# JuanDuGit/DH3D

Hardware: AMD Instinct MI355X
Metric: point-clouds/sec (higher is better)
Workload: dtype f32; 1 GPU; local-descriptor forward (basic_config), N=8192 K=8, batch=8; clouds_per_gpu=8, clouds_total=8, points=8192, knn=8, parallelism=clouds sharded over 1 GPU(s), no data-path collective, weights=random-init (no checkpoint blobs exist upstream), steps_in_flight=4

## Files before the change

### dh3d_amd/csrc/spatial.hip

```cpp
#include <math.h>

#include "cell_grid.h"
#include "common.h"
#include "wave_ops.h"

namespace {

constexpr int kThreads = 1024;
constexpr int kWaves = 16;

__device__ __forceinline__ unsigned spread6(unsigned v) {
  v &= 63u;
  v = (v | (v << 8)) & 0x300Fu;
  v = (v | (v << 4)) & 0x30C3u;
  v = (v | (v << 2)) & 0x9249u;
  return v;
}
constexpr unsigned kSchedCube = 0x186186u;

__device__ __forceinline__ unsigned deal_grid_bits(const float ext[3], int nb[3]) {
  float c0 = ext[0], c1 = ext[1], c2 = ext[2];
  int n0 = 0, n1 = 0, n2 = 0;
  unsigned sched = 0;
#pragma unroll
  for (int s = 0; s < 12; ++s) {
    int a = -1;
    float best = -1.f;
    if (n2 < 6) { a = 2; best = c2; }
    if (n1 < 6 && (a < 0 || c1 > best * 1.25f)) { best = a < 0 ? c1 : fmaxf(best, c1); a = 1; }
    if (n0 < 6 && (a < 0 || c0 > best * 1.25f)) { best = a < 0 ? c0 : fmaxf(best, c0); a = 0; }
    n0 += (int)(a == 0); n1 += (int)(a == 1); n2 += (int)(a == 2);
    c0 = a == 0 ? c0 * 0.5f : c0; c1 = a == 1 ? c1 * 0.5f : c1; c2 = a == 2 ? c2 * 0.5f : c2;
    sched |= (unsigned)a << (2 * s);
  }
  nb[0] = n0; nb[1] = n1; nb[2] = n2;
  return sched;
}

template <int PPT>
__global__ __launch_bounds__(kThreads) void spatial_sort_kernel(const float *__restrict__ xyz, int N,
                                                               int npad, float4 *__restrict__ sorted,
                                                               float *__restrict__ gbox, int *__restrict__ cells,
                                                               int occ_min) {
  extern __shared__ __attribute__((aligned(16))) unsigned s_raw[];
  unsigned *s_hist = s_raw + 2 * npad;
  float *s_red = reinterpret_cast<float *>(s_hist + kWaves * 64);
  unsigned *s_tab = reinterpret_cast<unsigned *>(s_red + 6 * kWaves);
  const int b = blockIdx.x, tid = threadIdx.x, lane = tid & 63;
  const int wave = __builtin_amdgcn_readfirstlane(tid >> 6);
  const float *pc = xyz + (size_t)b * N * 3;
  const int NG = (N + 63) / 64;

  const int SEG = npad / kWaves;
  float lo[3] = {INFINITY, INFINITY, INFINITY}, hi[3] = {-INFINITY, -INFINITY, -INFINITY};
  float px[PPT], py[PPT], pz[PPT];
#pragma unroll
  for (int j = 0; j < PPT; ++j) {
    const int k = min(wave * SEG + j * 64 + lane, N - 1);
    px[j] = pc[(size_t)k * 3]; py[j] = pc[(size_t)k * 3 + 1]; pz[j] = pc[(size_t)k * 3 + 2];
  }
#pragma unroll
  for (int j = 0; j < PPT; ++j) {
    lo[0] = fminf(lo[0], px[j]); hi[0] = fmaxf(hi[0], px[j]);
    lo[1] = fminf(lo[1], py[j]); hi[1] = fmaxf(hi[1], py[j]);
    lo[2] = fminf(lo[2], pz[j]); hi[2] = fmaxf(hi[2], pz[j]);
  }
#pragma unroll
  for (int a = 0; a < 3; ++a) {
    const float wl = wave_min_f32(lo[a]), wh = wave_max_f32(hi[a]);
    if (lane == 0) { s_red[wave * 6 + a] = wl; s_red[wave * 6 + 3 + a] = wh; }
  }
  __syncthreads();
  float scale[3], ext[3];
#pragma unroll
  for (int a = 0; a < 3; ++a) {
    float l = INFINITY, h = -INFINITY;
    for (int w = 0; w < kWaves; ++w) { l = fminf(l, s_red[w * 6 + a]); h = fmaxf(h, s_red[w * 6 + 3 + a]); }
    lo[a] = l;
    ext[a] = h - l;
  }
  int nb[3];
  const unsigned sched = deal_grid_bits(ext, nb);
#pragma unroll
  for (int a = 0; a < 3; ++a) scale[a] = (float)(4 << nb[a]) / fmaxf(ext[a], 1e-30f);
  if (cells && tid == 0) {
    int *ct = cells + (size_t)b * kCellInts;
    float *hd = reinterpret_cast<float *>(ct) + kCellHead;
    hd[0] = lo[0]; hd[1] = lo[1]; hd[2] = lo[2];
    hd[3] = scale[0]; hd[4] = scale[1]; hd[5] = scale[2];
    ct[kCellSched] = (int)sched;
  }
  const bool cube = sched == kSchedCube;
  if (!cube) {
    if (tid < 768) {
      const int a = tid >> 8;
      s_tab[tid] = cell_deposit(sched, a, tid & 255, 18, nb[a] + 2, 17);
    }
    __syncthreads();
  }
  constexpr bool RELOAD = PPT >= 16;
  unsigned key[PPT];
  const int q0 = (4 << nb[0]) - 1, q1 = (4 << nb[1]) - 1, q2 = (4 << nb[2]) - 1;
#pragma unroll
  for (int j0 = 0; j0 < PPT; j0 += 4) {
    float rx[4], ry[4], rz[4];
#pragma unroll
    for (int u = 0; u < 4; ++u) {
      if (j0 + u >= PPT) continue;
      if (RELOAD) {
        const int k = min(wave * SEG + (j0 + u) * 64 + lane, N - 1);
        rx[u] = pc[(size_t)k * 3]; ry[u] = pc[(size_t)k * 3 + 1]; rz[u] = pc[(size_t)k * 3 + 2];
      } else {
        rx[u] = px[j0 + u]; ry[u] = py[j0 + u]; rz[u] = pz[j0 + u];
      }
    }
#pragma unroll
    for (int u = 0; u < 4; ++u) {
      if (j0 + u >= PPT) continue;
      const int k = wave * SEG + (j0 + u) * 64 + lane;
      const unsigned cx = (unsigned)min(q0, max(0, (int)((rx[u] - lo[0]) * scale[0])));
      const unsigned cy = (unsigned)min(q1, max(0, (int)((ry[u] - lo[1]) * scale[1])));
      const unsigned cz = (unsigned)min(q2, max(0, (int)((rz[u] - lo[2]) * scale[2])));
      const unsigned cell = cube ? spread6(cx) | (spread6(cy) << 1) | (spread6(cz) << 2)
                                 : s_tab[cx] | s_tab[256 + cy] | s_tab[512 + cz];
      key[j0 + u] = k < N ? (cell << 14) | (unsigned)k : 0xFFFFFFFFu;
    }
    if (RELOAD) __builtin_amdgcn_sched_barrier(0);
  }
  unsigned *src = s_raw, *dst = s_raw + npad;
  const unsigned long long lt_mask = (1ull << lane) - 1ull;
  for (int pass = 0; pass < 3; ++pass) {
    const int shift = 14 + 6 * pass;
    s_hist[tid] = 0u;
    __syncthreads();
    unsigned local[PPT];
    unsigned *whist = s_hist + wave * 64;
#pragma unroll
    for (int j = 0; j < PPT; ++j) {
      const unsigned d = (key[j] >> shift) & 63u;
      unsigned long long same = ~0ull;
#pragma unroll
      for (int i = 0; i < 6; ++i) {
        const bool bit = (d >> i) & 1u;
        const unsigned long long bal = __ballot(bit);
        same &= bit ? bal : ~bal;
      }
      const unsigned before = whist[d];
      const unsigned rank = (unsigned)__popcll(same & lt_mask);
      local[j] = before + rank;
      if (rank == 0) whist[d] = before + (unsigned)__popcll(same);
    }
    __syncthreads();
    {
      const int d = tid >> 4, w = tid & 15;
      const unsigned v = s_hist[w * 64 + d];
      unsigned inc = v;
#pragma unroll
      for (int off = 1; off < 64; off <<= 1) {
        const unsigned up = __shfl_up(inc, off, 64);
        if (lane >= off) inc += up;
      }
      __syncthreads();
      if (lane == 63) s_red[wave] = __uint_as_float(inc);
      __syncthreads();
      unsigned base = 0;
      for (int ww = 0; ww < wave; ++ww) base += __float_as_uint(s_red[ww]);
      s_hist[w * 64 + d] = base + inc - v;
    }
    __syncthreads();
#pragma unroll
    for (int j = 0; j < PPT; ++j) {
      const unsigned d = (key[j] >> shift) & 63u;
      dst[whist[d] + local[j]] = key[j];
    }
    __syncthreads();
#pragma unroll
    for (int j = 0; j < PPT; ++j) key[j] = dst[wave * SEG + j * 64 + lane];
    unsigned *t = src; src = dst; dst = t;
  }
  const unsigned *s_keys = src;
  float gx[PPT], gy[PPT], gz[PPT];
  int gk[PPT];
#pragma unroll
  for (int j = 0; j < PPT; ++j) {
    const int i = min((wave + kWaves * j) * 64 + lane, N - 1);
    gk[j] = (int)(s_keys[i] & 0x3FFFu);
  }
#pragma unroll
  for (int j = 0; j < PPT; ++j) {
    gx[j] = pc[(size_t)gk[j] * 3]; gy[j] = pc[(size_t)gk[j] * 3 + 1]; gz[j] = pc[(size_t)gk[j] * 3 + 2];
  }
#pragma unroll
  for (int j = 0; j < PPT; ++j) {
    const int g = wave + kWaves * j;
    const int i = g * 64 + lane;
    const float x = gx[j], y = gy[j], z = gz[j];
    float lx = INFINITY, ly = INFINITY, lz = INFINITY, hx = -INFINITY, hy = -INFINITY, hz = -INFINITY;
    if (i < N) {
      sorted[(size_t)b * N + i] = make_float4(x, y, z, __int_as_float(gk[j]));
      lx = hx = x; ly = hy = y; lz = hz = z;
    }
    if (g < NG) {
      lx = wave_min_f32(lx); ly = wave_min_f32(ly); lz = wave_min_f32(lz);
      hx = wave_max_f32(hx); hy = wave_max_f32(hy); hz = wave_max_f32(hz);
      if (lane == 0) {
        float *o = gbox + ((size_t)b * NG + g) * 8;
        o[0] = lx; o[1] = ly; o[2] = lz; o[3] = 0.f; o[4] = hx; o[5] = hy; o[6] = hz; o[7] = 0.f;
      }
    }
  }
  if (cells) {
    int *ct = cells + (size_t)b * kCellInts;
#pragma unroll
    for (int j = 0; j < PPT; ++j) {
      const int i = wave * SEG + j * 64 + lane;
      if (i < N) {
        const int cur = (int)(s_keys[i] >> 20), prev = i > 0 ? (int)(s_keys[i - 1] >> 20) : -1;
        for (int c = prev + 1; c <= cur; ++c) ct[c] = i;
        if (i == N - 1)
          for (int c = cur + 1; c <= kGridCells; ++c) ct[c] = N;
      }
    }
    int occupied = 0;
#pragma unroll
    for (int j = 0; j < PPT; ++j) {
      const int i = wave * SEG + j * 64 + lane;
      if (i < N) occupied += (int)(i == 0 || (s_keys[i] >> 20) != (s_keys[i - 1] >> 20));
    }
#pragma unroll
    for (int off = 32; off > 0; off >>= 1) occupied += __shfl_xor(occupied, off, 64);
    __shared__ int s_occupied;
    if (tid == 0) s_occupied = 0;
    __syncthreads();
    if (lane == 0) atomicAdd(&s_occupied, occupied);
    __syncthreads();
    if (tid == 0) ct[kCellFlag] = s_occupied < occ_min ? 1 : 0;
  }
}

template <int PPT>
int sort_launch(const float *xyz, int B, int N, float4 *sorted, float *gbox, int *cells, hipStream_t s) {
  int npad = 2;
  while (npad < N) npad <<= 1;
  if (npad < 64 * kWaves) npad = 64 * kWaves;
  const size_t lds = sizeof(unsigned) * (2 * (size_t)npad + kWaves * 64 + 3 * 256) + sizeof(float) * 6 * kWaves;
  DH3D_ALLOW_BIG_LDS((spatial_sort_kernel<PPT>));
  const int occ_min = (int)(0.6 * kGridCells * (1.0 - exp(-(double)N / kGridCells)));
  hipLaunchKernelGGL((spatial_sort_kernel<PPT>), dim3(B), dim3(kThreads), lds, s, xyz, N, npad, sorted, gbox, cells,
                     occ_min);
  return dh3d_launch_status();
}

}

static int spatial_sort_any(const float *xyz, int B, int N, float *sorted, float *gbox, int *cells, void *stream) {
  DH3D_REQUIRE(xyz && sorted && gbox && B > 0 && N > 0);
  DH3D_SUPPORTED(N <= 16384);
  hipStream_t s = (hipStream_t)stream;
  float4 *so = reinterpret_cast<float4 *>(sorted);
  if (N <= 1024) return sort_launch<1>(xyz, B, N, so, gbox, cells, s);
  if (N <= 2048) return sort_launch<2>(xyz, B, N, so, gbox, cells, s);
  if (N <= 4096) return sort_launch<4>(xyz, B, N, so, gbox, cells, s);
  if (N <= 8192) return sort_launch<8>(xyz, B, N, so, gbox, cells, s);
  return sort_launch<16>(xyz, B, N, so, gbox, cells, s);
}

DH3D_API int dh3d_spatial_sort(const float *xyz, int B, int N, float *sorted, float *gbox, void *stream) {
  return spatial_sort_any(xyz, B, N, sorted, gbox, nullptr, stream);
}

DH3D_API int dh3d_spatial_sort_cells(const float *xyz, int B, int N, float *sorted, float *gbox, int32_t *cells, void *stream) {
  DH3D_REQUIRE(cells);
  return spatial_sort_any(xyz, B, N, sorted, gbox, cells, stream);
}
```

### dh3d_amd/csrc/flex_x6.hip

```cpp
#include <type_traits>

#include "bf16x3.h"

namespace {

typedef float f32x2 __attribute__((ext_vector_type(2)));
typedef float f32x4 __attribute__((ext_vector_type(4)));
constexpr int kTM = 32;
constexpr int kPPR = 32;
constexpr int kProducers = 8 * 64, kThreads = kProducers + 256;

template <int DIN, int DOUT>
struct X6Cfg {
  static constexpr int KD = 4 * DIN;
  static constexpr int LD = KD + 8;
  static constexpr int KB = KD / 16;
  static constexpr int KBH = KB / 2;
  static constexpr int VEC = DIN / 16;
  static constexpr int ROUNDS = kTM / kPPR;
  static constexpr int A_ELEMS = 3 * kTM * LD;
  static constexpr int P_FLOATS = 4 * 8 * 64;
  static constexpr int B3_VEC = 2 * KB * 64;
  static constexpr size_t LDS_BYTES = (size_t)2 * A_ELEMS * 2 + (size_t)2 * P_FLOATS * 4 + (size_t)B3_VEC * 16;
  static_assert(DOUT == 64 && (VEC == 2 || VEC == 4) && KBH % 2 == 0 && LDS_BYTES <= 159 * 1024, "shape");
};

__device__ __forceinline__ void wg_barrier(int = 0) { asm volatile("s_waitcnt lgkmcnt(0)\n\ts_barrier" ::: "memory"); }

template <int K>
__device__ __forceinline__ float row_bcast(float v) {
  return __builtin_bit_cast(float, __builtin_amdgcn_mov_dpp(__builtin_bit_cast(int, v), 0x150 + K, 0xf, 0xf, false));
}

__device__ __forceinline__ float hi16_of(float a) { return __uint_as_float(__float_as_uint(a) & 0xFFFF0000u); }

__device__ __forceinline__ void split3x2(const f32x2 v, unsigned &c1, unsigned &c2, unsigned &c3) {
  const float r0 = v[0] - hi16_of(v[0]), r1 = v[1] - hi16_of(v[1]);
  const float t0 = r0 - hi16_of(r0), t1 = r1 - hi16_of(r1);
  c1 = pack_hi16(v[0], v[1]);
  c2 = pack_hi16(r0, r1);
  c3 = pack_hi16(t0, t1);
}

template <int VEC> struct LaneVec;
template <> struct LaneVec<4> { typedef float4 type; };
template <> struct LaneVec<2> { typedef float2 type; };

template <int DIN, int DOUT, bool RAGGED>
__global__ __launch_bounds__(kThreads) void flex_conv_x6_kernel(
    const float *__restrict__ feat, const float *__restrict__ xyz, const int32_t *__restrict__ nbr,
    const uint4 *__restrict__ wp3, unsigned R, unsigned N, EpilogueArgs ep, float *__restrict__ out, int T) {
  using C = X6Cfg<DIN, DOUT>;
  using FV = typename LaneVec<C::VEC>::type;
  extern __shared__ __attribute__((aligned(16))) unsigned char s_raw[];
  unsigned short *s_A = reinterpret_cast<unsigned short *>(s_raw);
  float *s_P = reinterpret_cast<float *>(s_raw + (size_t)2 * C::A_ELEMS * 2);
  const int tid = threadIdx.x;
  const int wave = __builtin_amdgcn_readfirstlane(tid >> 6);
  const int x = blockIdx.x & 7, slot = blockIdx.x >> 3, S = gridDim.x >> 3;
  const int Tx = (T + 7) >> 3;
  const int tbeg = x * Tx + slot;
  const int tend = (x + 1) * Tx < T ? (x + 1) * Tx : T;
  const int cnt = tbeg < tend ? (tend - tbeg + S - 1) / S : 0;
  if (cnt == 0) return;

  if (wave < kProducers / 64) {
    __builtin_amdgcn_s_setprio(3);
    const int prow = tid >> 4, lj = tid & 15;
    const int c0 = lj * C::VEC;
    const unsigned mrec = (unsigned)(0x100000000ULL / N);
    const int G = cnt * C::ROUNDS;
    int nid[2][8], myid[2][2];
    FV fv[2][8];
    float qd[2][2], pcd[2];
    const int da = (tid >> 2) & 3, di = tid & 3;
    const int dcomp = di > 0 ? di - 1 : 0;

    auto row_of = [&](int g, unsigned &n, bool &ok) {
      const int i = g / C::ROUNDS, r = g % C::ROUNDS;
      n = (unsigned)(tbeg + i * S) * kTM + r * kPPR + prow;
      ok = (int)(g < G) & (int)(n < R);
      n = ok ? n : 0u;
    };
    auto issue_ids = [&](int s, int g) {
      unsigned n; bool ok;
      row_of(g, n, ok);
      const int4 *ip = reinterpret_cast<const int4 *>(nbr + (size_t)n * 8);
      const int4 a = ip[0], b = ip[1];
      nid[s][0] = a.x; nid[s][1] = a.y; nid[s][2] = a.z; nid[s][3] = a.w;
      nid[s][4] = b.x; nid[s][5] = b.y; nid[s][6] = b.z; nid[s][7] = b.w;
      myid[s][0] = nbr[(size_t)n * 8 + da];
      myid[s][1] = nbr[(size_t)n * 8 + 4 + da];
    };
    auto issue_feat = [&](int s, int g) {
      unsigned n; bool ok;
      row_of(g, n, ok);
      unsigned q = __umulhi(n, mrec);
      if (n - q * N >= N) ++q;
      const unsigned cloud0 = q * N;
      pcd[s] = xyz[(size_t)n * 3 + dcomp];
      qd[s][0] = *reinterpret_cast<const float *>(reinterpret_cast<const char *>(xyz) + (size_t)((cloud0 + (unsigned)myid[s][0]) * 12u + (unsigned)dcomp * 4u));
      qd[s][1] = *reinterpret_cast<const float *>(reinterpret_cast<const char *>(xyz) + (size_t)((cloud0 + (unsigned)myid[s][1]) * 12u + (unsigned)dcomp * 4u));
#pragma unroll
      for (int k = 0; k < 8; ++k) {
        const unsigned g2 = cloud0 + (unsigned)nid[s][k];
        fv[s][k] = *reinterpret_cast<const FV *>(reinterpret_cast<const char *>(feat) +
                                                 (size_t)(g2 * (unsigned)(DIN * 4) + (unsigned)(c0 * 4)));
      }
    };
    auto compute = [&](int s, int g) {
      const int i = g / C::ROUNDS, r = g % C::ROUNDS;
      float d0 = qd[s][0] - pcd[s], d1 = qd[s][1] - pcd[s];
      asm volatile("s_nop 1" : "+v"(d0), "+v"(d1));
      f32x2 acc[4][C::VEC / 2];
#define DH3D_X6_FMAC_BCAST(ACC, D, F, L) \
  asm("v_fmac_f32_dpp %0, %1, %2 row_newbcast:" #L " row_mask:0xf bank_mask:0xf" : "+v"(ACC) : "v"(D), "v"(F))
#define DH3D_X6_MUL_BCAST(ACC, D, F, L) \
  asm("v_mul_f32_dpp %0, %1, %2 row_newbcast:" #L " row_mask:0xf bank_mask:0xf" : "=v"(ACC) : "v"(D), "v"(F))
#define DH3D_X6_NEIGHBOUR_(KI, DS, LX, LY, LZ)                                                                   \
  {                                                                                                              \
    const float *fp = reinterpret_cast<const float *>(&fv[s][KI]);                                               \
    _Pragma("unroll") for (int h = 0; h < C::VEC / 2; ++h) {                                                     \
      _Pragma("unroll") for (int e = 0; e < 2; ++e) {                                                            \
        const float f = fp[2 * h + e];                                                                           \
        if ((KI) == 0) {                                                    \
          acc[0][h][e] = f;                                                                                      \
          DH3D_X6_MUL_BCAST(acc[1][h][e], DS, f, LX);                                                            \
          DH3D_X6_MUL_BCAST(acc[2][h][e], DS, f, LY);                                                            \
          DH3D_X6_MUL_BCAST(acc[3][h][e], DS, f, LZ);                                                            \
        } else {                                                                                                 \
          acc[0][h][e] += f;                                                                                     \
          DH3D_X6_FMAC_BCAST(acc[1][h][e], DS, f, LX);                                                           \
          DH3D_X6_FMAC_BCAST(acc[2][h][e], DS, f, LY);                                                           \
          DH3D_X6_FMAC_BCAST(acc[3][h][e], DS, f, LZ);                                                           \
        }                                                                                                        \
      }                                                                                                          \
    }                                                                                                            \
  }
#define DH3D_X6_NEIGHBOUR(KI)                                                                                    \
  if (((KI) & 3) == 0) DH3D_X6_NEIGHBOUR_(KI, ((KI) < 4 ? d0 : d1), 1, 2, 3)                                      \
  else if (((KI) & 3) == 1) DH3D_X6_NEIGHBOUR_(KI, ((KI) < 4 ? d0 : d1), 5, 6, 7)                                 \
  else if (((KI) & 3) == 2) DH3D_X6_NEIGHBOUR_(KI, ((KI) < 4 ? d0 : d1), 9, 10, 11)                               \
  else DH3D_X6_NEIGHBOUR_(KI, ((KI) < 4 ? d0 : d1), 13, 14, 15)
      DH3D_X6_NEIGHBOUR(0) DH3D_X6_NEIGHBOUR(1) DH3D_X6_NEIGHBOUR(2) DH3D_X6_NEIGHBOUR(3)
      DH3D_X6_NEIGHBOUR(4) DH3D_X6_NEIGHBOUR(5) DH3D_X6_NEIGHBOUR(6) DH3D_X6_NEIGHBOUR(7)
#undef DH3D_X6_NEIGHBOUR
#undef DH3D_X6_NEIGHBOUR_
#undef DH3D_X6_FMAC_BCAST
#undef DH3D_X6_MUL_BCAST
      unsigned short *row = s_A + (size_t)(i & 1) * C::A_ELEMS + (size_t)(r * kPPR + prow) * C::LD + c0;
#pragma unroll
      for (int c = 0; c < 4; ++c) {
        unsigned c1[C::VEC / 2], c2[C::VEC / 2], c3[C::VEC / 2];
#pragma unroll
        for (int h = 0; h < C::VEC / 2; ++h) {
          split3x2(acc[c][h], c1[h], c2[h], c3[h]);
        }
        if (C::VEC == 4) {
          *reinterpret_cast<uint2 *>(row + c * DIN) = make_uint2(c1[0], c1[C::VEC / 2 - 1]);
          *reinterpret_cast<uint2 *>(row + c * DIN + kTM * C::LD) = make_uint2(c2[0], c2[C::VEC / 2 - 1]);
          *reinterpret_cast<uint2 *>(row + c * DIN + 2 * kTM * C::LD) = make_uint2(c3[0], c3[C::VEC / 2 - 1]);
        } else {
          *reinterpret_cast<unsigned *>(row + c * DIN) = c1[0];
          *reinterpret_cast<unsigned *>(row + c * DIN + kTM * C::LD) = c2[0];
          *reinterpret_cast<unsigned *>(row + c * DIN + 2 * kTM * C::LD) = c3[0];
        }
      }
    };

    if ((wave >> 2) & 1) {
      issue_ids(0, 0);
      issue_ids(1, 1);
      issue_feat(0, 0);
      issue_ids(0, 2);
      for (int g = 0; g < G; g += 2) {
#pragma unroll
        for (int s = 0; s < 2; ++s) {
          const int gg = g + s;
          issue_feat(s ^ 1, gg + 1);
          issue_ids(s ^ 1, gg + 3);
          compute(s, gg);
          if (gg % C::ROUNDS == C::ROUNDS - 1 && gg < G) wg_barrier(gg / C::ROUNDS);
        }
      }
    } else {
      issue_ids(0, 0);
      issue_ids(1, 1);
      issue_feat(0, 0);
      issue_ids(0, 2);
      issue_feat(1, 1);
      issue_ids(1, 3);
      for (int g = 0; g < G; g += 2) {
#pragma unroll
        for (int s = 0; s < 2; ++s) {
          const int gg = g + s;
          compute(s, gg);
          issue_feat(s, gg + 2);
          issue_ids(s, gg + 4);
          if (gg % C::ROUNDS == C::ROUNDS - 1 && gg < G) wg_barrier(gg / C::ROUNDS);
        }
      }
    }
    wg_barrier(cnt);
  } else {
    const int cw = wave - kProducers / 64, lane = tid & 63;
    const int cb = cw & 1, kh = cw >> 1;
    uint4 breg[C::KBH][2];
    uint4 *const s_b3 = reinterpret_cast<uint4 *>(s_raw + (size_t)2 * C::A_ELEMS * 2 + (size_t)2 * C::P_FLOATS * 4) +
                        (size_t)(cb * C::KB + kh * C::KBH) * 64 + lane;
#pragma unroll
    for (int kb = 0; kb < C::KBH; ++kb) {
#pragma unroll
      for (int p = 0; p < 2; ++p)
        breg[kb][p] = wp3[((size_t)(cb * C::KB + kh * C::KBH + kb) * 3 + p) * 64 + lane];
      s_b3[(size_t)kb * 64] = wp3[((size_t)(cb * C::KB + kh * C::KBH + kb) * 3 + 2) * 64 + lane];
    }
    const int col = cb * 32 + (lane & 31);
    float sc = 1.f, sh = 0.f;
    if (ep.scale) sc = ep.scale[col];
    if (ep.shift) sh = ep.shift[col];
    if (ep.pre_bias) sh = fmaf(ep.pre_bias[col], sc, sh);
    const int lo = ep.act == DH3D_ACT_RELU ? 0 : INT_MIN;
    float4 *const s_P4 = reinterpret_cast<float4 *>(s_P);
    float4 *const p_mine = s_P4 + (size_t)(cw * 2) * 64 + lane;
    const float4 *const p_partner = s_P4 + (size_t)((cw ^ 2) * 2) * 64 + lane;
    const unsigned voff = (unsigned)(((4 * (lane >> 5) + 16 * kh) * DOUT + col) * 4);
    float keep[8];
    const unsigned short *const abase0 = s_A + (size_t)(lane & 31) * C::LD + 8 * (lane >> 5) + kh * C::KBH * 16;

    auto tile = [&](int i, auto prev_tag) {
      constexpr bool PREV = decltype(prev_tag)::value;
      const unsigned short *abase = abase0 + (size_t)(i & 1) * C::A_ELEMS;
      f32x16 acc0, acc1;
#pragma unroll
      for (int r = 0; r < 16; ++r) acc0[r] = acc1[r] = 0.f;
      bf16x8 a[2][3];
      uint4 b3r[2];
      float4 pp[2];
#pragma unroll
      for (int p = 0; p < 3; ++p) a[0][p] = *reinterpret_cast<const bf16x8 *>(abase + p * kTM * C::LD);
      b3r[0] = s_b3[0];
      if (PREV) {
        pp[0] = p_partner[(size_t)((i - 1) & 1) * 512];
        pp[1] = p_partner[(size_t)((i - 1) & 1) * 512 + 64];
      }
      float *const orow = reinterpret_cast<float *>(reinterpret_cast<char *>(out + (size_t)(tbeg + (i - 1) * S) * kTM * DOUT) + voff);
      const unsigned grow_prev = (unsigned)(tbeg + (i - 1) * S) * kTM + 4 * (lane >> 5) + 16 * kh;
      __builtin_amdgcn_sched_barrier(0);
#pragma unroll
      for (int kb = 0; kb < C::KBH; ++kb) {
        if (kb + 1 < C::KBH) {
#pragma unroll
          for (int p = 0; p < 3; ++p)
            a[(kb + 1) & 1][p] = *reinterpret_cast<const bf16x8 *>(abase + p * kTM * C::LD + (kb + 1) * 16);
          b3r[(kb + 1) & 1] = s_b3[(size_t)(kb + 1) * 64];
        }
        const bf16x8 a1 = a[kb & 1][0], a2 = a[kb & 1][1], a3 = a[kb & 1][2];
        const bf16x8 b1 = __builtin_bit_cast(bf16x8, breg[kb][0]), b2 = __builtin_bit_cast(bf16x8, breg[kb][1]),
                     b3 = __builtin_bit_cast(bf16x8, b3r[kb & 1]);
        acc0 = __builtin_amdgcn_mfma_f32_32x32x16_bf16(a3, b1, acc0, 0, 0, 0);
        acc1 = __builtin_amdgcn_mfma_f32_32x32x16_bf16(a1, b3, acc1, 0, 0, 0);
        acc0 = __builtin_amdgcn_mfma_f32_32x32x16_bf16(a2, b2, acc0, 0, 0, 0);
        acc1 = __builtin_amdgcn_mfma_f32_32x32x16_bf16(a2, b1, acc1, 0, 0, 0);
        acc0 = __builtin_amdgcn_mfma_f32_32x32x16_bf16(a1, b2, acc0, 0, 0, 0);
        acc1 = __builtin_amdgcn_mfma_f32_32x32x16_bf16(a1, b1, acc1, 0, 0, 0);
        if (PREV) {
#pragma unroll
          for (int jj = 0; jj < 8 / C::KBH; ++jj) {
            const int j = (8 / C::KBH) * kb + jj;
            const float part = reinterpret_cast<const float *>(&pp[j >> 2])[j & 3];
            const int vi = max(__float_as_int(fmaf(keep[j] + part, sc, sh)), lo);
            const int rowoff = (j & 3) + 8 * (j >> 2);
            if (!RAGGED || grow_prev + rowoff < R) reinterpret_cast<int *>(orow)[rowoff * DOUT] = vi;
          }
        }
        __builtin_amdgcn_sched_group_barrier(0x100, 4, 0);
#pragma unroll
        for (int m = 0; m < 6; ++m) {
          __builtin_amdgcn_sched_group_barrier(0x008, 1, 0);
          __builtin_amdgcn_sched_group_barrier(0x002, 1, 0);
          if (m % 3 == 2) __builtin_amdgcn_sched_group_barrier(0x040, 1, 0);
        }
        __builtin_amdgcn_sched_barrier(0);
      }
      float sum[16];
#pragma unroll
      for (int r = 0; r < 16; ++r) sum[r] = acc0[r] + acc1[r];
#pragma unroll
      for (int j = 0; j < 8; ++j) keep[j] = kh ? sum[8 + j] : sum[j];
      p_mine[(size_t)(i & 1) * 512] = kh ? make_float4(sum[0], sum[1], sum[2], sum[3]) : make_float4(sum[8], sum[9], sum[10], sum[11]);
      p_mine[(size_t)(i & 1) * 512 + 64] = kh ? make_float4(sum[4], sum[5], sum[6], sum[7]) : make_float4(sum[12], sum[13], sum[14], sum[15]);
    };

    wg_barrier(0);
    tile(0, std::false_type{});
    wg_barrier(1);
    for (int i = 1; i < cnt; ++i) {
      tile(i, std::true_type{});
      wg_barrier(i + 1);
    }
    {
      const int i = cnt;
      const float4 pp0 = p_partner[(size_t)((i - 1) & 1) * 512], pp1 = p_partner[(size_t)((i - 1) & 1) * 512 + 64];
      float *const orow = reinterpret_cast<float *>(reinterpret_cast<char *>(out + (size_t)(tbeg + (i - 1) * S) * kTM * DOUT) + voff);
      const unsigned grow_prev = (unsigned)(tbeg + (i - 1) * S) * kTM + 4 * (lane >> 5) + 16 * kh;
#pragma unroll
      for (int j = 0; j < 8; ++j) {
        const float part = j < 4 ? reinterpret_cast<const float *>(&pp0)[j & 3] : reinterpret_cast<const float *>(&pp1)[j & 3];
        const int vi = max(__float_as_int(fmaf(keep[j] + part, sc, sh)), lo);
        const int rowoff = (j & 3) + 8 * (j >> 2);
        if (!RAGGED || grow_prev + rowoff < R) reinterpret_cast<int *>(orow)[rowoff * DOUT] = vi;
      }
    }
  }
}

__global__ __launch_bounds__(256) void pack_flex_weight_x3_kernel(const float *__restrict__ theta,
                                                                 const float *__restrict__ bias, int Din, int Dout,
                                                                 unsigned short *__restrict__ packed) {
  const int Kd = 4 * Din, KB = Kd / 16;
  const long long total = (long long)Kd * Dout;
  for (long long e = (long long)blockIdx.x * 256 + threadIdx.x; e < total; e += (long long)gridDim.x * 256) {
    const int j = (int)(e & 7);
    const int lane = (int)((e >> 3) & 63);
    const long long blk = e >> 9;
    const int kb = (int)(blk % KB), nb = (int)(blk / KB);
    const int k = kb * 16 + 8 * (lane >> 5) + j, col = nb * 32 + (lane & 31);
    const int comp = k / Din, i = k % Din;
    const float w = comp == 0 ? bias[(size_t)i * Dout + col] : theta[((size_t)(comp - 1) * Din + i) * Dout + col];
    unsigned c1, c2, c3;
    split3(w, c1, c2, c3);
    const size_t base = ((size_t)blk * 3) * 512 + (size_t)lane * 8 + j;
    packed[base] = (unsigned short)c1;
    packed[base + 512] = (unsigned short)c2;
    packed[base + 1024] = (unsigned short)c3;
  }
}

int persistent_grid() {
  static int g = 0;
  if (g == 0) {
    int dev = 0, cus = 0;
    if (hipGetDevice(&dev) != hipSuccess || hipDeviceGetAttribute(&cus, hipDeviceAttributeMultiprocessorCount, dev) != hipSuccess)
      cus = 256;
    g = cus >= 8 ? (cus & ~7) : 8;
  }
  return g;
}

template <int DIN, int DOUT>
int flex_conv_x6_launch(const float *feat, const float *xyz, const int32_t *nbr, const void *wp3, int B, int N,
                        const EpilogueArgs &ep, float *out, hipStream_t s, int reserve_per_xcd) {
  using C = X6Cfg<DIN, DOUT>;
  const long long R = (long long)B * N;
  const int T = dh3d_cdiv(R, kTM);
  int grid = persistent_grid() - 8 * (reserve_per_xcd > 0 ? reserve_per_xcd : 0);
  grid = grid < 8 ? 8 : grid;
  if (R % kTM == 0) {
    auto kern = flex_conv_x6_kernel<DIN, DOUT, false>;
    DH3D_ALLOW_BIG_LDS(kern);
    hipLaunchKernelGGL(kern, dim3(grid), dim3(kThreads), C::LDS_BYTES, s, feat, xyz, nbr,
                       static_cast<const uint4 *>(wp3), (unsigned)R, (unsigned)N, ep, out, T);
  } else {
    auto kern = flex_conv_x6_kernel<DIN, DOUT, true>;
    DH3D_ALLOW_BIG_LDS(kern);
    hipLaunchKernelGGL(kern, dim3(grid), dim3(kThreads), C::LDS_BYTES, s, feat, xyz, nbr,
                       static_cast<const uint4 *>(wp3), (unsigned)R, (unsigned)N, ep, out, T);
  }
  return dh3d_launch_status();
}

}

DH3D_API int dh3d_pack_flex_weight_x3(const float *theta, const float *bias, int Din, int Dout, void *packed,
                                      void *stream) {
  DH3D_REQUIRE(theta && bias && packed && Din > 0 && Dout > 0);
  DH3D_SUPPORTED(Din % 4 == 0 && Dout % 32 == 0);
  hipLaunchKernelGGL(pack_flex_weight_x3_kernel, dim3(dh3d_cdiv((long long)4 * Din * Dout, 256)), dim3(256), 0,
                     (hipStream_t)stream, theta, bias, Din, Dout, static_cast<unsigned short *>(packed));
  return dh3d_launch_status();
}

DH3D_API int dh3d_flex_conv_pm_x6_fwd_r(const float *features, const float *xyz, const int32_t *nbr,
                                        const void *wpacked_x3, int B, int N, int K, int Din, int Dout,
                                        const dh3d_epilogue *ep, int reserve_cus_per_xcd, float *out, void *stream) {
  DH3D_REQUIRE(features && xyz && nbr && wpacked_x3 && out && B > 0 && N > 0 && K > 0);
  DH3D_REQUIRE(reserve_cus_per_xcd >= 0 && reserve_cus_per_xcd < 32);
  const long long R = (long long)B * N;
  DH3D_SUPPORTED((!ep || ep->act != DH3D_ACT_SIGMOID) && K == 8 && N >= 2 && R * Din * 4 < (1LL << 32) && R + kTM < (1LL << 31));
  const EpilogueArgs e = dh3d_ep(ep);
  hipStream_t s = (hipStream_t)stream;
  if (Din == 32 && Dout == 64)
    return flex_conv_x6_launch<32, 64>(features, xyz, nbr, wpacked_x3, B, N, e, out, s, reserve_cus_per_xcd);
  if (Din == 64 && Dout == 64)
    return flex_conv_x6_launch<64, 64>(features, xyz, nbr, wpacked_x3, B, N, e, out, s, reserve_cus_per_xcd);
  return DH3D_ERR_UNSUPPORTED;
}

DH3D_API int dh3d_flex_conv_pm_x6_fwd(const float *features, const float *xyz, const int32_t *nbr,
                                      const void *wpacked_x3, int B, int N, int K, int Din, int Dout,
                                      const dh3d_epilogue *ep, float *out, void *stream) {
  return dh3d_flex_conv_pm_x6_fwd_r(features, xyz, nbr, wpacked_x3, B, N, K, Din, Dout, ep, 0, out, stream);
}
```

Measured before the change: 40720 point-clouds/sec.

## Replace three-pass radix sort with cell counting sort split across blocks

```diff
diff --git a/dh3d_amd/csrc/spatial.hip b/dh3d_amd/csrc/spatial.hip
--- a/dh3d_amd/csrc/spatial.hip
+++ b/dh3d_amd/csrc/spatial.hip
@@ -1,5 +1,6 @@
 #include <math.h>
 
+#include "block_ops.h"
 #include "cell_grid.h"
 #include "common.h"
 #include "wave_ops.h"
@@ -8,6 +9,8 @@
 
 constexpr int kThreads = 1024;
 constexpr int kWaves = 16;
+constexpr int kOwn = 1024;
+constexpr unsigned kCellMax = 512;
 
 __device__ __forceinline__ unsigned spread6(unsigned v) {
   v &= 63u;
@@ -43,14 +46,21 @@
                                                                float *__restrict__ gbox, int *__restrict__ cells,
                                                                int occ_min) {
   extern __shared__ __attribute__((aligned(16))) unsigned s_raw[];
-  unsigned *s_hist = s_raw + 2 * npad;
-  float *s_red = reinterpret_cast<float *>(s_hist + kWaves * 64);
+  unsigned *s_keys = s_raw;
+  unsigned *s_cnt = s_keys + npad;
+  unsigned *s_hist = s_cnt;
+  unsigned *s_T = s_cnt + kGridCells;
+  unsigned *s_own = s_T + kGridCells + 4;
+  float *s_red = reinterpret_cast<float *>(s_own + kOwn);
   unsigned *s_tab = reinterpret_cast<unsigned *>(s_red + 6 * kWaves);
-  const int b = blockIdx.x, tid = threadIdx.x, lane = tid & 63;
+  int *s_w = reinterpret_cast<int *>(s_tab + 3 * 256);
+  const int b = blockIdx.x, part = blockIdx.y, tid = threadIdx.x, lane = tid & 63;
   const int wave = __builtin_amdgcn_readfirstlane(tid >> 6);
   const float *pc = xyz + (size_t)b * N * 3;
   const int NG = (N + 63) / 64;
-
+  const int own_lo = part * kOwn, own_hi = min(own_lo + kOwn, N);
+
+  reinterpret_cast<uint4 *>(s_cnt)[tid] = make_uint4(0u, 0u, 0u, 0u);
   const int SEG = npad / kWaves;
   float lo[3] = {INFINITY, INFINITY, INFINITY}, hi[3] = {-INFINITY, -INFINITY, -INFINITY};
   float px[PPT], py[PPT], pz[PPT];
@@ -83,8 +93,8 @@
   const unsigned sched = deal_grid_bits(ext, nb);
 #pragma unroll
   for (int a = 0; a < 3; ++a) scale[a] = (float)(4 << nb[a]) / fmaxf(ext[a], 1e-30f);
-  if (cells && tid == 0) {
-    int *ct = cells + (size_t)b * kCellInts;
+  int *ct = cells && part == 0 ? cells + (size_t)b * kCellInts : nullptr;
+  if (ct && tid == 0) {
     float *hd = reinterpret_cast<float *>(ct) + kCellHead;
     hd[0] = lo[0]; hd[1] = lo[1]; hd[2] = lo[2];
     hd[3] = scale[0]; hd[4] = scale[1]; hd[5] = scale[2];
@@ -124,117 +134,120 @@
       const unsigned cell = cube ? spread6(cx) | (spread6(cy) << 1) | (spread6(cz) << 2)
                                  : s_tab[cx] | s_tab[256 + cy] | s_tab[512 + cz];
       key[j0 + u] = k < N ? (cell << 14) | (unsigned)k : 0xFFFFFFFFu;
+      if (k < N) atomicAdd(&s_cnt[cell >> 6], 1u);
     }
     if (RELOAD) __builtin_amdgcn_sched_barrier(0);
   }
-  unsigned *src = s_raw, *dst = s_raw + npad;
-  const unsigned long long lt_mask = (1ull << lane) - 1ull;
-  for (int pass = 0; pass < 3; ++pass) {
-    const int shift = 14 + 6 * pass;
-    s_hist[tid] = 0u;
+  __syncthreads();
+  bool crowded_cell = false;
+  {
+    const uint4 c = reinterpret_cast<const uint4 *>(s_cnt)[tid];
+    const int mine = (int)(c.x + c.y + c.z + c.w) + (((int)(c.x != 0u) + (int)(c.y != 0u) + (int)(c.z != 0u) + (int)(c.w != 0u)) << 16);
+    int total;
+    uint4 t;
+    t.x = (unsigned)block_excl_scan<kThreads>(mine, s_w, total) & 0xFFFFu;
+    t.y = t.x + c.x; t.z = t.y + c.y; t.w = t.z + c.z;
+    reinterpret_cast<uint4 *>(s_T)[tid] = t;
+    if (tid == 0) s_T[kGridCells] = (unsigned)N;
+    if (ct) {
+      if (tid == 0) { ct[kGridCells] = N; ct[kCellFlag] = (total >> 16) < occ_min ? 1 : 0; }
+    }
+    const unsigned lo_u = (unsigned)own_lo, hi_u = (unsigned)own_hi;
+    crowded_cell = (c.x > kCellMax && t.x < hi_u && t.y > lo_u) || (c.y > kCellMax && t.y < hi_u && t.z > lo_u) ||
+                   (c.z > kCellMax && t.z < hi_u && t.w > lo_u) || (c.w > kCellMax && t.w < hi_u && t.w + c.w > lo_u);
+  }
+  const unsigned *s_mine;
+  const bool ranked = !__syncthreads_or(crowded_cell);
+  if (ct) {
+#pragma unroll
+    for (int j = 0; j < kGridCells / kThreads; ++j) ct[j * kThreads + tid] = (int)s_T[j * kThreads + tid];
+  }
+  if (ranked) {
+#pragma unroll
+    for (int j = 0; j < PPT; ++j) {
+      const unsigned c = key[j] >> 20;
+      if (wave * SEG + j * 64 + lane < N) s_keys[s_T[c] + atomicSub(&s_cnt[c], 1u) - 1u] = key[j];
+    }
     __syncthreads();
-    unsigned local[PPT];
-    unsigned *whist = s_hist + wave * 64;
-#pragma unroll
-    for (int j = 0; j < PPT; ++j) {
-      const unsigned d = (key[j] >> shift) & 63u;
-      unsigned long long same = ~0ull;
-#pragma unroll
-      for (int i = 0; i < 6; ++i) {
-        const bool bit = (d >> i) & 1u;
-        const unsigned long long bal = __ballot(bit);
-        same &= bit ? bal : ~bal;
-      }
-      const unsigned before = whist[d];
-      const unsigned rank = (unsigned)__popcll(same & lt_mask);
-      local[j] = before + rank;
-      if (rank == 0) whist[d] = before + (unsigned)__popcll(same);
+    const int first = (int)s_T[s_keys[own_lo] >> 20], end = (int)s_T[(s_keys[own_hi - 1] >> 20) + 1];
+    for (int s = first + tid; s < end; s += kThreads) {
+      const unsigned k0 = s_keys[s];
+      const int a = (int)s_T[k0 >> 20], e = (int)s_T[(k0 >> 20) + 1];
+      int p = a;
+      for (int q = a; q < e; ++q) p += (int)(s_keys[q] < k0);
+      if (p >= own_lo && p < own_hi) s_own[p - own_lo] = k0;
     }
     __syncthreads();
-    {
-      const int d = tid >> 4, w = tid & 15;
-      const unsigned v = s_hist[w * 64 + d];
-      unsigned inc = v;
-#pragma unroll
-      for (int off = 1; off < 64; off <<= 1) {
-        const unsigned up = __shfl_up(inc, off, 64);
-        if (lane >= off) inc += up;
-      }
-      __syncthreads();
-      if (lane == 63) s_red[wave] = __uint_as_float(inc);
-      __syncthreads();
-      unsigned base = 0;
-      for (int ww = 0; ww < wave; ++ww) base += __float_as_uint(s_red[ww]);
-      s_hist[w * 64 + d] = base + inc - v;
-    }
-    __syncthreads();
-#pragma unroll
-    for (int j = 0; j < PPT; ++j) {
-      const unsigned d = (key[j] >> shift) & 63u;
-      dst[whist[d] + local[j]] = key[j];
-    }
-    __syncthreads();
-#pragma unroll
-    for (int j = 0; j < PPT; ++j) key[j] = dst[wave * SEG + j * 64 + lane];
-    unsigned *t = src; src = dst; dst = t;
-  }
-  const unsigned *s_keys = src;
-  float gx[PPT], gy[PPT], gz[PPT];
-  int gk[PPT];
-#pragma unroll
-  for (int j = 0; j < PPT; ++j) {
-    const int i = min((wave + kWaves * j) * 64 + lane, N - 1);
-    gk[j] = (int)(s_keys[i] & 0x3FFFu);
-  }
-#pragma unroll
-  for (int j = 0; j < PPT; ++j) {
-    gx[j] = pc[(size_t)gk[j] * 3]; gy[j] = pc[(size_t)gk[j] * 3 + 1]; gz[j] = pc[(size_t)gk[j] * 3 + 2];
-  }
-#pragma unroll
-  for (int j = 0; j < PPT; ++j) {
-    const int g = wave + kWaves * j;
-    const int i = g * 64 + lane;
-    const float x = gx[j], y = gy[j], z = gz[j];
-    float lx = INFINITY, ly = INFINITY, lz = INFINITY, hx = -INFINITY, hy = -INFINITY, hz = -INFINITY;
-    if (i < N) {
-      sorted[(size_t)b * N + i] = make_float4(x, y, z, __int_as_float(gk[j]));
-      lx = hx = x; ly = hy = y; lz = hz = z;
-    }
-    if (g < NG) {
-      lx = wave_min_f32(lx); ly = wave_min_f32(ly); lz = wave_min_f32(lz);
-      hx = wave_max_f32(hx); hy = wave_max_f32(hy); hz = wave_max_f32(hz);
-      if (lane == 0) {
-        float *o = gbox + ((size_t)b * NG + g) * 8;
-        o[0] = lx; o[1] = ly; o[2] = lz; o[3] = 0.f; o[4] = hx; o[5] = hy; o[6] = hz; o[7] = 0.f;
-      }
-    }
-  }
-  if (cells) {
-    int *ct = cells + (size_t)b * kCellInts;
-#pragma unroll
-    for (int j = 0; j < PPT; ++j) {
-      const int i = wave * SEG + j * 64 + lane;
-      if (i < N) {
-        const int cur = (int)(s_keys[i] >> 20), prev = i > 0 ? (int)(s_keys[i - 1] >> 20) : -1;
-        for (int c = prev + 1; c <= cur; ++c) ct[c] = i;
-        if (i == N - 1)
-          for (int c = cur + 1; c <= kGridCells; ++c) ct[c] = N;
-      }
-    }
-    int occupied = 0;
-#pragma unroll
-    for (int j = 0; j < PPT; ++j) {
-      const int i = wave * SEG + j * 64 + lane;
-      if (i < N) occupied += (int)(i == 0 || (s_keys[i] >> 20) != (s_keys[i - 1] >> 20));
-    }
-#pragma unroll
-    for (int off = 32; off > 0; off >>= 1) occupied += __shfl_xor(occupied, off, 64);
-    __shared__ int s_occupied;
-    if (tid == 0) s_occupied = 0;
-    __syncthreads();
-    if (lane == 0) atomicAdd(&s_occupied, occupied);
-    __syncthreads();
-    if (tid == 0) ct[kCellFlag] = s_occupied < occ_min ? 1 : 0;
+    s_mine = s_own;
+  } else {
+    const unsigned long long lt_mask = (1ull << lane) - 1ull;
+    for (int pass = 0; pass < 3; ++pass) {
+      const int shift = 14 + 6 * pass;
+      s_hist[tid] = 0u;
+      __syncthreads();
+      unsigned local[PPT];
+      unsigned *whist = s_hist + wave * 64;
+#pragma unroll
+      for (int j = 0; j < PPT; ++j) {
+        const unsigned d = (key[j] >> shift) & 63u;
+        unsigned long long same = ~0ull;
+#pragma unroll
+        for (int i = 0; i < 6; ++i) {
+          const bool bit = (d >> i) & 1u;
+          const unsigned long long bal = __ballot(bit);
+          same &= bit ? bal : ~bal;
+        }
+        const unsigned before = whist[d];
+        const unsigned rank = (unsigned)__popcll(same & lt_mask);
+        local[j] = before + rank;
+        if (rank == 0) whist[d] = before + (unsigned)__popcll(same);
+      }
+      __syncthreads();
+      {
+        const int d = tid >> 4, w = tid & 15;
+        const unsigned v = s_hist[w * 64 + d];
+        unsigned inc = v;
+#pragma unroll
+        for (int off = 1; off < 64; off <<= 1) {
+          const unsigned up = __shfl_up(inc, off, 64);
+          if (lane >= off) inc += up;
+        }
+        __syncthreads();
+        if (lane == 63) s_red[wave] = __uint_as_float(inc);
+        __syncthreads();
+        unsigned base = 0;
+        for (int ww = 0; ww < wave; ++ww) base += __float_as_uint(s_red[ww]);
+        s_hist[w * 64 + d] = base + inc - v;
+      }
+      __syncthreads();
+#pragma unroll
+      for (int j = 0; j < PPT; ++j) {
+        const unsigned d = (key[j] >> shift) & 63u;
+        s_keys[whist[d] + local[j]] = key[j];
+      }
+      __syncthreads();
+      if (pass < 2) {
+#pragma unroll
+        for (int j = 0; j < PPT; ++j) key[j] = s_keys[wave * SEG + j * 64 + lane];
+      }
+    }
+    s_mine = s_keys + own_lo;
+  }
+  const int g = part * (kOwn / 64) + wave, i = tid < kOwn ? g * 64 + lane : N;
+  float lx = INFINITY, ly = INFINITY, lz = INFINITY, hx = -INFINITY, hy = -INFINITY, hz = -INFINITY;
+  if (i < N) {
+    const int k = (int)(s_mine[tid] & 0x3FFFu);
+    const float x = pc[(size_t)k * 3], y = pc[(size_t)k * 3 + 1], z = pc[(size_t)k * 3 + 2];
+    sorted[(size_t)b * N + i] = make_float4(x, y, z, __int_as_float(k));
+    lx = hx = x; ly = hy = y; lz = hz = z;
+  }
+  if (tid < kOwn && g < NG) {
+    lx = wave_min_f32(lx); ly = wave_min_f32(ly); lz = wave_min_f32(lz);
+    hx = wave_max_f32(hx); hy = wave_max_f32(hy); hz = wave_max_f32(hz);
+    if (lane == 0) {
+      float *o = gbox + ((size_t)b * NG + g) * 8;
+      o[0] = lx; o[1] = ly; o[2] = lz; o[3] = 0.f; o[4] = hx; o[5] = hy; o[6] = hz; o[7] = 0.f;
+    }
   }
 }
 
@@ -243,10 +256,11 @@
   int npad = 2;
   while (npad < N) npad <<= 1;
   if (npad < 64 * kWaves) npad = 64 * kWaves;
-  const size_t lds = sizeof(unsigned) * (2 * (size_t)npad + kWaves * 64 + 3 * 256) + sizeof(float) * 6 * kWaves;
+  const size_t lds = sizeof(unsigned) * ((size_t)npad + 2 * kGridCells + 4 + kOwn + 3 * 256 + kWaves) + sizeof(float) * 6 * kWaves;
   DH3D_ALLOW_BIG_LDS((spatial_sort_kernel<PPT>));
   const int occ_min = (int)(0.6 * kGridCells * (1.0 - exp(-(double)N / kGridCells)));
-  hipLaunchKernelGGL((spatial_sort_kernel<PPT>), dim3(B), dim3(kThreads), lds, s, xyz, N, npad, sorted, gbox, cells,
+  const int G = (N + kOwn - 1) / kOwn;
+  hipLaunchKernelGGL((spatial_sort_kernel<PPT>), dim3(B, G), dim3(kThreads), lds, s, xyz, N, npad, sorted, gbox, cells,
                      occ_min);
   return dh3d_launch_status();
 }
```

After: 41100 point-clouds/sec (median of 6 runs). No clear change (+0.9%).

## Use 8-lane float4 producer groups with quad-perm broadcasts for narrow DIN

Applied to the files above, without the earlier changes.

```diff
diff --git a/dh3d_amd/csrc/flex_x6.hip b/dh3d_amd/csrc/flex_x6.hip
--- a/dh3d_amd/csrc/flex_x6.hip
+++ b/dh3d_amd/csrc/flex_x6.hip
@@ -16,13 +16,15 @@
   static constexpr int LD = KD + 8;
   static constexpr int KB = KD / 16;
   static constexpr int KBH = KB / 2;
-  static constexpr int VEC = DIN / 16;
+  static constexpr int VEC = 4;
+  static constexpr int LPP = DIN / VEC;
+  static constexpr int NQ = LPP == 16 ? 2 : 8;
   static constexpr int ROUNDS = kTM / kPPR;
   static constexpr int A_ELEMS = 3 * kTM * LD;
   static constexpr int P_FLOATS = 4 * 8 * 64;
   static constexpr int B3_VEC = 2 * KB * 64;
   static constexpr size_t LDS_BYTES = (size_t)2 * A_ELEMS * 2 + (size_t)2 * P_FLOATS * 4 + (size_t)B3_VEC * 16;
-  static_assert(DOUT == 64 && (VEC == 2 || VEC == 4) && KBH % 2 == 0 && LDS_BYTES <= 159 * 1024, "shape");
+  static_assert(DOUT == 64 && (LPP == 8 || LPP == 16) && KBH % 2 == 0 && LDS_BYTES <= 159 * 1024, "shape");
 };
 
 __device__ __forceinline__ void wg_barrier(int = 0) { asm volatile("s_waitcnt lgkmcnt(0)\n\ts_barrier" ::: "memory"); }
@@ -42,16 +44,13 @@
   c3 = pack_hi16(t0, t1);
 }
 
-template <int VEC> struct LaneVec;
-template <> struct LaneVec<4> { typedef float4 type; };
-template <> struct LaneVec<2> { typedef float2 type; };
-
 template <int DIN, int DOUT, bool RAGGED>
 __global__ __launch_bounds__(kThreads) void flex_conv_x6_kernel(
     const float *__restrict__ feat, const float *__restrict__ xyz, const int32_t *__restrict__ nbr,
     const uint4 *__restrict__ wp3, unsigned R, unsigned N, EpilogueArgs ep, float *__restrict__ out, int T) {
   using C = X6Cfg<DIN, DOUT>;
-  using FV = typename LaneVec<C::VEC>::type;
+  typedef float4 FV;
+  constexpr bool QUAD = C::LPP == 8;
   extern __shared__ __attribute__((aligned(16))) unsigned char s_raw[];
   unsigned short *s_A = reinterpret_cast<unsigned short *>(s_raw);
   float *s_P = reinterpret_cast<float *>(s_raw + (size_t)2 * C::A_ELEMS * 2);
@@ -66,18 +65,19 @@
 
   if (wave < kProducers / 64) {
     __builtin_amdgcn_s_setprio(3);
-    const int prow = tid >> 4, lj = tid & 15;
+    const int grp = QUAD ? wave >> 2 : 0;
+    const int prow = QUAD ? (tid & 255) >> 3 : tid >> 4, lj = tid & (C::LPP - 1);
     const int c0 = lj * C::VEC;
     const unsigned mrec = (unsigned)(0x100000000ULL / N);
-    const int G = cnt * C::ROUNDS;
+    const int G = QUAD ? (cnt + 1 - grp) >> 1 : cnt * C::ROUNDS;
     int nid[2][8], myid[2][2];
     FV fv[2][8];
-    float qd[2][2], pcd[2];
+    float qd[2][C::NQ], pcd[2];
     const int da = (tid >> 2) & 3, di = tid & 3;
     const int dcomp = di > 0 ? di - 1 : 0;
 
     auto row_of = [&](int g, unsigned &n, bool &ok) {
-      const int i = g / C::ROUNDS, r = g % C::ROUNDS;
+      const int i = QUAD ? 2 * g + grp : g / C::ROUNDS, r = QUAD ? 0 : g % C::ROUNDS;
       n = (unsigned)(tbeg + i * S) * kTM + r * kPPR + prow;
       ok = (int)(g < G) & (int)(n < R);
       n = ok ? n : 0u;
@@ -89,8 +89,10 @@
       const int4 a = ip[0], b = ip[1];
       nid[s][0] = a.x; nid[s][1] = a.y; nid[s][2] = a.z; nid[s][3] = a.w;
       nid[s][4] = b.x; nid[s][5] = b.y; nid[s][6] = b.z; nid[s][7] = b.w;
-      myid[s][0] = nbr[(size_t)n * 8 + da];
-      myid[s][1] = nbr[(size_t)n * 8 + 4 + da];
+      if constexpr (!QUAD) {
+        myid[s][0] = nbr[(size_t)n * 8 + da];
+        myid[s][1] = nbr[(size_t)n * 8 + 4 + da];
+      }
     };
     auto issue_feat = [&](int s, int g) {
       unsigned n; bool ok;
@@ -99,8 +101,12 @@
       if (n - q * N >= N) ++q;
       const unsigned cloud0 = q * N;
       pcd[s] = xyz[(size_t)n * 3 + dcomp];
-      qd[s][0] = *reinterpret_cast<const float *>(reinterpret_cast<const char *>(xyz) + (size_t)((cloud0 + (unsigned)myid[s][0]) * 12u + (unsigned)dcomp * 4u));
-      qd[s][1] = *reinterpret_cast<const float *>(reinterpret_cast<const char *>(xyz) + (size_t)((cloud0 + (unsigned)myid[s][1]) * 12u + (unsigned)dcomp * 4u));
+      const int *cid = QUAD ? nid[s] : myid[s];
+#pragma unroll
+      for (int k = 0; k < C::NQ; ++k) {
+        const unsigned g2 = cloud0 + (unsigned)cid[k];
+        qd[s][k] = *reinterpret_cast<const float *>(reinterpret_cast<const char *>(xyz) + (size_t)(g2 * 12u + (unsigned)dcomp * 4u));
+      }
 #pragma unroll
       for (int k = 0; k < 8; ++k) {
         const unsigned g2 = cloud0 + (unsigned)nid[s][k];
@@ -109,14 +115,19 @@
       }
     };
     auto compute = [&](int s, int g) {
-      const int i = g / C::ROUNDS, r = g % C::ROUNDS;
-      float d0 = qd[s][0] - pcd[s], d1 = qd[s][1] - pcd[s];
-      asm volatile("s_nop 1" : "+v"(d0), "+v"(d1));
+      const int i = QUAD ? 2 * g + grp : g / C::ROUNDS, r = QUAD ? 0 : g % C::ROUNDS;
+      float d[C::NQ];
+#pragma unroll
+      for (int k = 0; k < C::NQ; ++k) d[k] = qd[s][k] - pcd[s];
+      if constexpr (QUAD)
+        asm volatile("s_nop 1" : "+v"(d[0]), "+v"(d[1]), "+v"(d[2]), "+v"(d[3]), "+v"(d[4]), "+v"(d[5]), "+v"(d[6]), "+v"(d[7]));
+      else
+        asm volatile("s_nop 1" : "+v"(d[0]), "+v"(d[1]));
       f32x2 acc[4][C::VEC / 2];
 #define DH3D_X6_FMAC_BCAST(ACC, D, F, L) \
-  asm("v_fmac_f32_dpp %0, %1, %2 row_newbcast:" #L " row_mask:0xf bank_mask:0xf" : "+v"(ACC) : "v"(D), "v"(F))
+  asm("v_fmac_f32_dpp %0, %1, %2 " L " row_mask:0xf bank_mask:0xf" : "+v"(ACC) : "v"(D), "v"(F))
 #define DH3D_X6_MUL_BCAST(ACC, D, F, L) \
-  asm("v_mul_f32_dpp %0, %1, %2 row_newbcast:" #L " row_mask:0xf bank_mask:0xf" : "=v"(ACC) : "v"(D), "v"(F))
+  asm("v_mul_f32_dpp %0, %1, %2 " L " row_mask:0xf bank_mask:0xf" : "=v"(ACC) : "v"(D), "v"(F))
 #define DH3D_X6_NEIGHBOUR_(KI, DS, LX, LY, LZ)                                                                   \
   {                                                                                                              \
     const float *fp = reinterpret_cast<const float *>(&fv[s][KI]);                                               \
@@ -138,10 +149,11 @@
     }                                                                                                            \
   }
 #define DH3D_X6_NEIGHBOUR(KI)                                                                                    \
-  if (((KI) & 3) == 0) DH3D_X6_NEIGHBOUR_(KI, ((KI) < 4 ? d0 : d1), 1, 2, 3)                                      \
-  else if (((KI) & 3) == 1) DH3D_X6_NEIGHBOUR_(KI, ((KI) < 4 ? d0 : d1), 5, 6, 7)                                 \
-  else if (((KI) & 3) == 2) DH3D_X6_NEIGHBOUR_(KI, ((KI) < 4 ? d0 : d1), 9, 10, 11)                               \
-  else DH3D_X6_NEIGHBOUR_(KI, ((KI) < 4 ? d0 : d1), 13, 14, 15)
+  if constexpr (QUAD) DH3D_X6_NEIGHBOUR_(KI, d[KI], "quad_perm:[1,1,1,1]", "quad_perm:[2,2,2,2]", "quad_perm:[3,3,3,3]") \
+  else if (((KI) & 3) == 0) DH3D_X6_NEIGHBOUR_(KI, d[(KI) >> 2], "row_newbcast:1", "row_newbcast:2", "row_newbcast:3")   \
+  else if (((KI) & 3) == 1) DH3D_X6_NEIGHBOUR_(KI, d[(KI) >> 2], "row_newbcast:5", "row_newbcast:6", "row_newbcast:7")   \
+  else if (((KI) & 3) == 2) DH3D_X6_NEIGHBOUR_(KI, d[(KI) >> 2], "row_newbcast:9", "row_newbcast:10", "row_newbcast:11") \
+  else DH3D_X6_NEIGHBOUR_(KI, d[(KI) >> 2], "row_newbcast:13", "row_newbcast:14", "row_newbcast:15")
       DH3D_X6_NEIGHBOUR(0) DH3D_X6_NEIGHBOUR(1) DH3D_X6_NEIGHBOUR(2) DH3D_X6_NEIGHBOUR(3)
       DH3D_X6_NEIGHBOUR(4) DH3D_X6_NEIGHBOUR(5) DH3D_X6_NEIGHBOUR(6) DH3D_X6_NEIGHBOUR(7)
 #undef DH3D_X6_NEIGHBOUR
@@ -156,18 +168,34 @@
         for (int h = 0; h < C::VEC / 2; ++h) {
           split3x2(acc[c][h], c1[h], c2[h], c3[h]);
         }
-        if (C::VEC == 4) {
-          *reinterpret_cast<uint2 *>(row + c * DIN) = make_uint2(c1[0], c1[C::VEC / 2 - 1]);
-          *reinterpret_cast<uint2 *>(row + c * DIN + kTM * C::LD) = make_uint2(c2[0], c2[C::VEC / 2 - 1]);
-          *reinterpret_cast<uint2 *>(row + c * DIN + 2 * kTM * C::LD) = make_uint2(c3[0], c3[C::VEC / 2 - 1]);
-        } else {
-          *reinterpret_cast<unsigned *>(row + c * DIN) = c1[0];
-          *reinterpret_cast<unsigned *>(row + c * DIN + kTM * C::LD) = c2[0];
-          *reinterpret_cast<unsigned *>(row + c * DIN + 2 * kTM * C::LD) = c3[0];
-        }
+        *reinterpret_cast<uint2 *>(row + c * DIN) = make_uint2(c1[0], c1[1]);
+        *reinterpret_cast<uint2 *>(row + c * DIN + kTM * C::LD) = make_uint2(c2[0], c2[1]);
+        *reinterpret_cast<uint2 *>(row + c * DIN + 2 * kTM * C::LD) = make_uint2(c3[0], c3[1]);
       }
     };
 
+    if constexpr (QUAD) {
+      issue_ids(0, 0);
+      issue_ids(1, 1);
+      issue_feat(0, 0);
+      issue_ids(0, 2);
+      if (grp) wg_barrier(0);
+      auto round = [&](int s, int gg) {
+        compute(s, gg);
+        wg_barrier(2 * gg + grp);
+        issue_feat(s ^ 1, gg + 1);
+        issue_ids(s ^ 1, gg + 3);
+        wg_barrier(2 * gg + grp + 1);
+      };
+      int g = 0;
+      for (; g + 1 < G; g += 2) {
+        round(0, g);
+        round(1, g + 1);
+      }
+      if (g < G) round(0, g);
+      if ((cnt & 1) == grp) wg_barrier(cnt);
+      return;
+    }
     if ((wave >> 2) & 1) {
       issue_ids(0, 0);
       issue_ids(1, 1);
```

Result: faster. 40470 point-clouds/sec before, 41060 point-clouds/sec after (median of 6 runs) (+1.5%).
